# amolchanov86/gym_art

Hardware: AMD Instinct MI355X
Metric: env-steps/sec (whole node) at N=2^20 Hummingbird; achieved HBM GB/s (higher is better)
Workload: dtype f64

## Files before the change

gym_art_amd/_lib.py:

```python
import ctypes as C
import os

import numpy as np

_HERE = os.path.dirname(os.path.abspath(__file__))
LIB_PATH = os.environ.get("GAQ_LIB") or os.path.join(_HERE, "libgaq.so")
ABI_VERSION = 5
STATE_PLANES = 42
AUX_WORDS = 17

CTRL_RAW_ZERO_MIDDLE, CTRL_RAW, CTRL_MELLINGER = 0, 1, 2
NOISE_OFF, NOISE_PHILOX, NOISE_INPUT = 0, 1, 2
REW_QUADROTOR, REW_MULTI_LOG = 0, 1
OBS_BODY_FRAME, OBS_APPEND_H, OBS_APPEND_ACC, OBS_APPEND_ACT = 1, 2, 4, 8
OBS_QUAT, OBS_APPEND_T2W, OBS_APPEND_T2T = 16, 32, 64


class GaqModel(C.Structure):
    _fields_ = [("mass", C.c_double), ("inertia", C.c_double * 3), ("thrust_max", C.c_double * 4),
                ("torque_max", C.c_double * 4), ("prop_pos", C.c_double * 12), ("damp_time_up", C.c_double),
                ("damp_time_down", C.c_double), ("linearity", C.c_double), ("arm", C.c_double),
                ("ou_sigma", C.c_double), ("vel_damp", C.c_double), ("damp_omega_quadratic", C.c_double),
                ("c_drag", C.c_double), ("c_roll", C.c_double)]

# ... 195 lines not shown
    ("gaq_get_aux", C.c_int, [_P, _P]),
    ("gaq_get_state", C.c_int, [_P, _P]),
    ("gaq_set_state", C.c_int, [_P, _P]),
    ("gaq_observe", C.c_int, [_P, _P]),
    ("gaq_done_list", C.c_int, [_P, _P, C.c_int64, C.POINTER(C.c_int64)]),
    ("gaq_set_terminal_obs_dev", C.c_int, [_P, _P]),
    ("gaq_track_episodes", C.c_int, [_P, C.c_int32]),
    ("gaq_episode_stats", C.c_int, [_P, C.POINTER(C.c_int64), C.POINTER(C.c_double), C.POINTER(C.c_double),
                                    C.POINTER(C.c_double), C.c_int32]),
    ("gaq_pack_rows_dev", C.c_int, [_P, _P, _P, _P, _P, _P]),
    ("gaq_set_packed_rows_dev", C.c_int, [_P, _P]),
    ("gaq_nan_count", C.c_int, [_P, C.POINTER(C.c_int64)]),
    ("gaq_last_kernel_ms", C.c_int, [_P, C.POINTER(C.c_float)]),
    ("gaq_set_graph_safe", C.c_int, [_P, C.c_int32]),
    ("gaq_uniform_counters", C.c_int, [_P, C.POINTER(C.c_int32), C.POINTER(C.c_uint32), C.POINTER(C.c_int32)]),
    ("gaq_set_timing", C.c_int, [_P, C.c_int32]),
    ("gaq_hbm_copy_dev", C.c_int, [_P, _P, C.c_size_t, _P]),
    ("gaq_synchronize", C.c_int, [_P]),
    ("gaq_stream", C.c_void_p, [_P]),
    ("gaq_create_sharded", C.c_int, [C.POINTER(GaqConfig), C.POINTER(C.c_int32), C.c_int32, C.POINTER(_P)]),
    ("gaq_sharded_from_handles", C.c_int, [C.POINTER(_P), C.c_int32, C.POINTER(_P)]),
    ("gaq_destroy_sharded", C.c_int, [_P]),
    ("gaq_sharded_num_shards", C.c_int, [_P]),
    ("gaq_sharded_shard", C.c_void_p, [_P, C.c_int32]),
    ("gaq_sharded_range", C.c_int, [_P, C.c_int32, C.POINTER(C.c_int64), C.POINTER(C.c_int64), C.POINTER(C.c_int32)]),
    ("gaq_sharded_num_envs", C.c_int64, [_P]),
    ("gaq_shard_range", C.c_int, [C.c_int64, C.c_int32, C.c_int32, C.c_int32, C.POINTER(C.c_int64), C.POINTER(C.c_int64)]),
    ("gaq_reset_sharded_dev", C.c_int, [_P, _P, _P, _P]),
    ("gaq_step_sharded_dev", C.c_int, [_P, _P, _P, _P, _P, _P]),
    ("gaq_reset_sharded", C.c_int, [_P, _P, _P]),
# ... 100 lines not shown
```

gym_art_amd/csrc/gaq.hip:

```cpp
#include "gaq_host.hpp"

#define GAQ_X(FEAT) extern template __global__ GAQ_STEP_SIG(FEAT)
GAQ_STEP_ALL(GAQ_X)
#undef GAQ_X
#define GAQ_X(FEAT) extern template __global__ GAQ_ROLL_SIG(FEAT)
GAQ_ROLL_ALL(GAQ_X)
#undef GAQ_X

namespace {

using namespace gaqk;

__global__ __launch_bounds__(kBlock) void episode_kernel(int64_t n, const float* __restrict__ reward,
                                                          const uint8_t* __restrict__ done, float* __restrict__ ep_ret,
                                                          uint32_t* __restrict__ ep_len, double* __restrict__ acc) {
  const int64_t i = (int64_t)blockIdx.x * kBlock + threadIdx.x;
  float ret = 0.0f; uint32_t len = 0; bool fin = false;
  if (i < n) {
    ret = ep_ret[i] + reward[i];
    len = ep_len[i] + 1u;
    fin = done[i] != 0;
    ep_ret[i] = fin ? 0.0f : ret;
    ep_len[i] = fin ? 0u : len;
  }
// ... 212 lines not shown
int svd_period_of(double dt) {
  double t = 0.0; int k = 0;
  while (!(t > 0.5)) { t += dt; ++k; if (k > 1000000) break; }
  return k;
}

}

int fail(int code, const std::string& msg) { g_err = msg; return code; }
int env_override(const char* name) { const char* v = getenv(name); return v ? (v[0] == '1' ? 1 : 0) : -1; }
LaunchRecord& launch_record() { static LaunchRecord r; return r; }

namespace {

Overrides read_overrides() {
  return {env_override("GAQ_FORCE_GENERIC") == 1, env_override("GAQ_NO_AUXP") == 1, env_override("GAQ_PREDRAW"), env_override("GAQ_NT"),
          env_override("GAQ_UNIFORM_CTR") != 0};
}
constexpr uint32_t kCtrGuard = 0xA5C3A5C3u;
constexpr int kCtrGuardWords = kTile;
constexpr int kSweepDefault = 1;

struct Layout { bool alias, pack, shadow, fp32; };
struct Selection { uint32_t variant; bool generic; int lds_per_wave; };
struct ParamFlags { bool lag, drag; };
struct Plan { Layout layout; Selection sel; };

bool step_instantiated(uint32_t f) {
  switch (f) {
#define GAQ_X(FEAT) case (FEAT):
    GAQ_STEP_ALL(GAQ_X)
#undef GAQ_X
// ... 363 lines not shown
  }
  const bool self_counting = (launch_variant & gaq::F_CTR) != 0;
  if (e->d.step_ctr && !self_counting) {
    bool capturing = false;
    hipStreamCaptureStatus cs = hipStreamCaptureStatusNone;
    if (hipStreamIsCapturing(st, &cs) == hipSuccess) capturing = cs == hipStreamCaptureStatusActive; else (void)hipGetLastError();
    if (e->ctr_spread || capturing) {
      hipLaunchKernelGGL(fold_counter_kernel, dim3(1), dim3(1), 0, st, e->d.step_ctr);
      HIP_TRY(hipGetLastError());
      if (!capturing) e->ctr_spread = false;
    }
  }
  if (launch_variant != e->noted_step) { launch_record().note(0, launch_variant); e->noted_step = launch_variant; }
#define GAQ_LAUNCH(FEAT) \
  hipLaunchKernelGGL(step_kernel<(FEAT)>, grid, block, lds, st, e->d, e->sc, e->um, actions, obs, reward, done, lpw)
  switch (launch_variant) {
#define GAQ_X(FEAT) case (int)(FEAT): GAQ_LAUNCH(FEAT); break;
    GAQ_STEP_ALL(GAQ_X)
#undef GAQ_X
    default: return fail(GAQ_ERR_STATE, "internal: no kernel instantiation for this feature mask");
  }
#undef GAQ_LAUNCH
  HIP_TRY(hipGetLastError());
  if (e->d.ep_ret) {
    const dim3 g2((unsigned)((e->d.n + kBlock - 1) / kBlock));
    hipLaunchKernelGGL(episode_kernel, g2, block, 0, st, e->d.n, reward, done, e->d.ep_ret, e->d.ep_len, e->d.ep_acc);
    HIP_TRY(hipGetLastError());
  }
  if (e->d.rz_every > 0 && e->d.jinv) { if (int rc = launch_jinv(e, st, done)) return rc; }
  if (e->d.rz_every > 0) {
    e->rz_since_refill += 1;
    const int period = e->sc.ep_len + 1 < 64 ? e->sc.ep_len + 1 : 64;
    if (e->d.step_ctr || e->rz_since_refill >= period) {
// ... 807 lines not shown
  if (!e) return fail(GAQ_ERR_INVALID, "null handle");
  if (valid_out) *valid_out = e->uni.valid ? 1 : 0;
  if (word_out) *word_out = e->uni.word;
  if (guard_intact_out) {
    HIP_TRY(hipSetDevice(e->cfg.device));
    HIP_TRY(hipStreamSynchronize(e->stream));
    if (int rc_ = sync_handle(e)) return rc_;
    uint32_t g[kCtrGuardWords];
    HIP_TRY(hipMemcpy(g, e->d.ctr + e->d.ntiles * kTile, sizeof(g), hipMemcpyDeviceToHost));
    *guard_intact_out = 1;
    for (uint32_t w : g) if (w != kCtrGuard) *guard_intact_out = 0;
  }
  return GAQ_OK;
}

int gaq_set_timing(gaq_env* e, int32_t enabled) {
  if (!e) return fail(GAQ_ERR_INVALID, "null handle");
  e->timing = enabled != 0; e->timed = false;
  return GAQ_OK;
}

int gaq_last_kernel_ms(gaq_env* e, float* ms_out) {
  if (!e || !ms_out) return fail(GAQ_ERR_INVALID, "null argument");
  if (!e->timed) return fail(GAQ_ERR_STATE, "no timed launch recorded (gaq_set_timing)");
  HIP_TRY(hipSetDevice(e->cfg.device));
  HIP_TRY(hipEventSynchronize(e->ev1));
  HIP_TRY(hipEventElapsedTime(ms_out, e->ev0, e->ev1));
  return GAQ_OK;
}

// ... 24 lines not shown
```

gym_art_amd/csrc/gaq_host.hpp:

```cpp
#pragma once

#include <hip/hip_runtime.h>

#include <algorithm>
#include <cmath>
#include <cstdio>
#include <cstdlib>
#include <cstring>
#include <functional>
#include <mutex>
#include <new>
#include <set>
#include <string>
#include <vector>

#include "gaq_kernels.hpp"
#include "../../include/gaq.h"

using namespace gaqk;

namespace {
struct Randomizer {
  int32_t sampler, every;
  double ratio[gaq::TL_COUNT];
  gaq::ParamTree base;
};
}

enum ParamFlag : uint8_t { PF_LAG = 1, PF_DRAG = 2, PF_NONCOMPACT = 4, PF_DAMP = 8 };
inline uint8_t param_flags(double tau_up, double tau_down, double c_drag, double c_roll, bool compact_ok, double vel_damp, double damp_q) {
  return (uint8_t)((!(tau_up >= 1.0 && tau_down >= 1.0) ? PF_LAG : 0) | ((c_drag != 0.0 || c_roll != 0.0) ? PF_DRAG : 0) |
                   (!compact_ok ? PF_NONCOMPACT : 0) | ((vel_damp != 0.0 || damp_q != 0.0) ? PF_DAMP : 0));
}

struct Overrides { bool force_generic = false, no_auxp = false; int predraw = -1, nt = -1; bool uniform_ctr = true; };

struct UniformCtr { bool eligible = false, valid = false, svd_known = false; uint32_t word = 0; };

struct gaq_env {
  gaq_config cfg;
  StepCfg sc;
  Model<double> um;
  DevPtrs d;
  int obs_dim = 18;
  hipStream_t stream = nullptr;
  hipEvent_t ev0 = nullptr, ev1 = nullptr;
  bool timing = false, timed = false;
  uint64_t reset_calls = 0;
  const float* noise_next = nullptr;
  uint32_t noted_step = 0xFFFFFFFFu, noted_roll = 0xFFFFFFFFu, noted_proll = 0xFFFFFFFFu;
// ... 88 lines not shown
```

gym_art_amd/csrc/gaq_inst.hip:

```cpp
#include "gaq_kernels.hpp"

#ifndef GAQ_PART
#error "compile with -DGAQ_PART=0 ... 7"
#endif
#define GAQ_CAT2(a, b) a##b
#define GAQ_CAT(a, b) GAQ_CAT2(a, b)
#define GAQ_X(FEAT) template __global__ GAQ_STEP_SIG(FEAT)
GAQ_CAT(GAQ_STEP_PART, GAQ_PART)(GAQ_X)
#undef GAQ_X
#define GAQ_X(FEAT) template __global__ GAQ_ROLL_SIG(FEAT)
GAQ_CAT(GAQ_ROLL_PART, GAQ_PART)(GAQ_X)
#undef GAQ_X
#define GAQ_X(FEAT) template __global__ GAQ_PROLL_SIG(FEAT)
GAQ_CAT(GAQ_PROLL_PART, GAQ_PART)(GAQ_X)
#undef GAQ_X
```

gym_art_amd/csrc/gaq_kernels.hpp:

```cpp
#pragma once

#include <hip/hip_runtime.h>

#include <cstddef>
#include <cstdint>

#include "../../include/gaq.h"
#include "quad_core.hpp"
#include "quad_params_dev.hpp"

namespace gaqk {

#ifndef GAQ_LD_AUX
#define GAQ_LD_AUX 0
#endif
#ifndef GAQ_ST_AUX
#define GAQ_ST_AUX 0
#endif
#ifndef GAQ_ACT_AUX
#define GAQ_ACT_AUX 0
#endif
#ifndef GAQ_ACTION_AUX
#define GAQ_ACTION_AUX GAQ_ACT_AUX
#endif
// ... 518 lines not shown
  __device__ __forceinline__ void neighbour(int j, const float* me, float* o) const {
    const int src = (int)((lane & ~(uint32_t)(agents - 1)) | ((lane + (uint32_t)j) & (uint32_t)(agents - 1)));
#pragma unroll
    for (int k = 0; k < 6; ++k) o[k] = __shfl(me[k], src);
  }
  __device__ __forceinline__ bool any(bool b) const { return __any(b) != 0; }
};

__device__ __forceinline__ void wait_dma() { asm volatile("s_waitcnt vmcnt(0)" ::: "memory"); }
__device__ __forceinline__ void wave_lds_fence() {
  __builtin_amdgcn_fence(__ATOMIC_RELEASE, "wavefront");
  __builtin_amdgcn_wave_barrier();
  __builtin_amdgcn_fence(__ATOMIC_ACQUIRE, "wavefront");
}

constexpr int kCtrSlots = 64;
constexpr int kCtrStride = 544;
__device__ __forceinline__ uint64_t step_counter_read(const DevPtrs& p, uint32_t lane) {
  static_assert(kCtrSlots == kTile, "one counter word per lane");
  return p.step_ctr[lane * kCtrStride];
}
__device__ __forceinline__ uint64_t step_counter_sum(uint64_t c) {
#pragma unroll
  for (int o = 1; o < kCtrSlots; o <<= 1) c += __shfl_xor(c, o);
  const uint32_t lo = __builtin_amdgcn_readfirstlane((uint32_t)c), hi = __builtin_amdgcn_readfirstlane((uint32_t)(c >> 32));
  return ((uint64_t)hi << 32) | lo;
}
__device__ __forceinline__ uint64_t step_counter_checkin(const DevPtrs& p, uint64_t raw, uint32_t lane) {
  const uint64_t c = step_counter_sum(raw);
  const uint32_t gwave = __builtin_amdgcn_readfirstlane(blockIdx.x * (uint32_t)(kBlock / kTile) + (threadIdx.x >> 6));
// ... 91 lines not shown
    asm("s_waitcnt lgkmcnt(0)" : "+s"(carry) : "s"(token), "s"(p.ntiles), "s"(p.n), "s"(p.step_ctr), "s"(p.ctr_shift), "s"(p.core), "s"(p.ctr),
        "s"(actions), "s"(lds_per_wave));
  }
  return carry;
}

template <uint32_t F> constexpr int kStepMinWaves = 1;
#ifndef GAQ_NO_FLOORS
template <> inline constexpr int kStepMinWaves<214036u> = 3;
template <> inline constexpr int kStepMinWaves<82962u> = 3;
#endif
constexpr uint32_t kXcds = 8;
template <uint32_t F> constexpr bool kSweeps = true;
template <> inline constexpr bool kSweeps<17428u> = false;
template <> inline constexpr bool kSweeps<2569u> = false;
template <uint32_t F>
__global__ __launch_bounds__(kBlock) __attribute__((amdgpu_waves_per_eu(kStepMinWaves<F>))) void step_kernel(DevPtrs p, StepCfg cfg, Model<double> um,
                                                       const float* __restrict__ actions, float* obs,
                                                       float* __restrict__ reward, uint8_t* __restrict__ done,
                                                       int lds_per_wave) {
  constexpr bool G = (F & gaq::F_GENERIC) != 0;
  constexpr bool A = (F & gaq::F_ALIAS) != 0;
  static_assert(!(G && A), "obs/state aliasing exists in the specialised kernels only");
  extern __shared__ __attribute__((aligned(16))) char smem[];
  int wave_ = __builtin_amdgcn_readfirstlane(threadIdx.x >> 6);
  if constexpr (kArgPrologue<F> != 0)
    wave_ = kernarg_batch<F, kArgPrologue<F>, kUniCtr<F>>(kernarg_warm(), wave_, p, actions, lds_per_wave, cfg.sweep);
  const int wave = wave_;
  bool uni = false;
  if constexpr (kUniCtr<F>) uni = ((uint32_t)cfg.sweep & gaq::kUniCtrValid) != 0;
  const uint32_t lane = threadIdx.x & 63u;
  uint32_t block = blockIdx.x;
  if constexpr ((F & gaq::F_CTR) == 0) {
    if (p.step_ctr) cfg.step_index = *p.step_ctr >> p.ctr_shift;
    if constexpr (kSweeps<F>) {
// ... 74 lines not shown
    if constexpr ((F & gaq::F_SWARM) != 0) {
      float* row = reinterpret_cast<float*>(rows) + lane * D;
      gaq::env_step<T, F>(s, *mp, cfg, act, cfg.env_offset + (uint64_t)i, [&](int, int) { return 0.0f; }, out,
                          [&](int k, float v, int) { row[k] = v; }, term_row, WaveSwarm{lane, cfg.swarm.agents});
    } else if constexpr (G) {
      const float* nz = p.noise_in;
      const int64_t n = p.n;
      float* row = reinterpret_cast<float*>(rows) + lane * D;
      if constexpr (kAuxRowsInLds) out.aux_row = reinterpret_cast<float*>(rows + aux_off) + lane * gaq::AUX_WORDS;
      const float* sz = p.sense_in;
      gaq::env_step<T, F>(s, *mp, cfg, act, cfg.env_offset + (uint64_t)i,
                               [&](int k, int c) { return nz[((int64_t)k * 4 + c) * n + i]; }, out,
                               [&](int k, float v, int) { row[k] = v; }, term_row, WaveSwarm{lane, cfg.swarm.agents},
                               [&](int c, int slot, int j) { return sz ? sz[((int64_t)(c * 12 + slot) * 3 + j) * n + i] : 0.0f; });
      if constexpr (gaq::kAux<F> && !kAuxRowsInLds) store_aux(p, i, out);
    } else if constexpr (gaq::kHeadsAreObs<F>) {
      gaq::env_step<T, F>(s, *mp, cfg, act, cfg.env_offset + (uint64_t)i, [&](int k, int c) { return k == 0 ? pre0[c] : pre1[c]; }, out,
                          [&](int, float, int) {}, term_row);
    } else if constexpr (kObsRowsInLds) {
      float* row = reinterpret_cast<float*>(rows) + lane * D;
      if constexpr (kAuxRowsInLds) out.aux_row = reinterpret_cast<float*>(rows + aux_off) + lane * gaq::AUX_WORDS;
      gaq::env_step<T, F>(s, *mp, cfg, act, cfg.env_offset + (uint64_t)i, [&](int, int) { return 0.0f; }, out,
                          [&](int k, float v, int) { row[k] = v; }, term_row);
      if constexpr (gaq::kAux<F> && !kAuxRowsInLds) store_aux(p, i, out);
    } else {
      gaq::env_step<T, F>(s, *mp, cfg, act, cfg.env_offset + (uint64_t)i, [&](int, int) { return 0.0f; }, out,
                          [&](int k, float v, int slot) { if (slot < 0) ob[k] = v; else ob[18 + slot] = v; }, term_row);
      if constexpr (gaq::kAux<F>) store_aux(p, i, out);
    }
  }
// ... 13 lines not shown
        (void)__builtin_amdgcn_raw_ptr_buffer_atomic_add_i32(1, rt, (uint32_t)i * 4u, third, 0);
        (void)__builtin_amdgcn_raw_ptr_buffer_atomic_add_i32(1, rt, (uint32_t)i * 4u, 2 * third, 0);
        s.svd_ctr = 0;
#pragma unroll
        for (int j = 0; j < 4; ++j) s.ou[j] = 0.0f;
      }
    }
  }
  if constexpr (kObsRowsInLds) {
    wave_lds_fence();
    if constexpr (A) flush_obs(p.obs_copy, p.n, D, tile, rows, lane);
    else flush_obs(obs, p.n, D, tile, rows, lane);
    if constexpr (kAuxRowsInLds) { if (p.aux) flush_obs(p.aux, p.n, gaq::AUX_WORDS, tile, rows + aux_off, lane); }
    wave_lds_fence();
  }
  write_image<F>(cfg, buf, lane, s);
  wave_lds_fence();
  stage_out<F>(p, cfg, tile, buf, lane, obs);
  if (!uni) {
    auto rc = __builtin_amdgcn_make_buffer_rsrc(p.ctr, 0, (int)(p.ntiles * kTile * 4), 0x00020000);
    __builtin_amdgcn_raw_buffer_store_b32((s.tick & 0xFFFFu) | (s.svd_ctr << 16), rc, (uint32_t)i * 4u, 0, kStAux<F>);
  }
  if (live) {
    if constexpr (GAQ_OUT_NT != 0) { __builtin_nontemporal_store(out.reward, &reward[i]); __builtin_nontemporal_store(out.done, &done[i]); }
    else { reward[i] = out.reward; done[i] = out.done; }
    if (!isfinite(out.reward)) atomicAdd(p.nan_count, 1u);
  }
  if constexpr (!gaq::kHeadsAreObs<F> && !kObsRowsInLds) {
    float* obs_rows_out = obs;
    if constexpr (A) obs_rows_out = p.obs_copy;
// ... 359 lines not shown
  policy_rollout_body<F>(p, cfg, um, T, obs, reward, done, smem, tile, lane, &pol, scratch, act_out);
}

}

#define GAQ_STEP_PART0(X) X(8u) X(1u) X(3u) X(16u) X(48u) X(2049u) X(2065u) X(3089u) X(2097u) X(4116u) X(8468u) X(16384u) X(33808u) X(197648u) X(459792u) X(197649u) X(199697u) X(16385u) X(16401u) X(18433u) X(18449u)
#define GAQ_STEP_PART1(X) X(9u) X(0u) X(2u) X(17u) X(49u) X(2051u) X(2067u) X(3091u) X(4244u) X(4372u) X(8470u) X(16386u) X(33810u) X(17424u) X(197650u) X(459794u) X(197651u) X(199699u) X(16387u) X(16403u) X(18435u) X(18451u)
#define GAQ_STEP_PART2(X) X(72u) X(2057u) X(4u) X(18u) X(50u) X(2053u) X(2069u) X(3093u) X(4500u) X(4118u) X(8471u) X(16388u) X(33812u) X(66578u) X(66583u) X(68625u) X(16389u) X(16405u) X(18437u) X(18453u)
#define GAQ_STEP_PART3(X) X(73u) X(2121u) X(5u) X(19u) X(51u) X(2055u) X(2071u) X(3095u) X(4246u) X(4374u) X(8596u) X(16390u) X(33814u) X(17426u) X(197652u) X(459796u) X(197653u) X(199701u) X(16391u) X(16407u) X(18439u) X(18455u)
#define GAQ_STEP_PART4(X) X(520u) X(6u) X(20u) X(52u) X(1040u) X(1041u) X(148u) X(276u) X(2099u) X(4502u) X(16400u) X(16402u) X(66576u) X(66581u) X(68627u) X(17425u) X(82960u) X(214032u) X(19473u)
#define GAQ_STEP_PART5(X) X(521u) X(7u) X(21u) X(53u) X(1042u) X(1043u) X(150u) X(278u) X(2101u) X(4119u) X(8598u) X(584u) X(17428u) X(197654u) X(459798u) X(197655u) X(199703u) X(17427u) X(82962u) X(214034u) X(19475u)
#define GAQ_STEP_PART6(X) X(2569u) X(22u) X(54u) X(1044u) X(1045u) X(151u) X(279u) X(404u) X(2103u) X(4247u) X(16404u) X(66580u) X(66577u) X(68631u) X(17429u) X(82964u) X(214036u) X(19477u)
#define GAQ_STEP_PART7(X) X(23u) X(55u) X(1046u) X(1047u) X(406u) X(407u) X(4375u) X(4503u) X(8599u) X(16406u) X(17430u) X(66582u) X(66579u) X(68629u) X(17431u) X(82966u) X(214038u) X(19479u)
#define GAQ_STEP_ALL(X) GAQ_STEP_PART0(X) GAQ_STEP_PART1(X) GAQ_STEP_PART2(X) GAQ_STEP_PART3(X) GAQ_STEP_PART4(X) GAQ_STEP_PART5(X) \
                        GAQ_STEP_PART6(X) GAQ_STEP_PART7(X)
#define GAQ_ROLL_PART0(X) X(16u) X(48u)
#define GAQ_ROLL_PART1(X) X(17u) X(49u)
#define GAQ_ROLL_PART2(X) X(18u) X(50u)
#define GAQ_ROLL_PART3(X) X(19u) X(51u)
#define GAQ_ROLL_PART4(X) X(20u) X(52u)
#define GAQ_ROLL_PART5(X) X(21u) X(53u)
#define GAQ_ROLL_PART6(X) X(22u) X(54u)
#define GAQ_ROLL_PART7(X) X(23u) X(55u)
#define GAQ_ROLL_ALL(X) GAQ_ROLL_PART0(X) GAQ_ROLL_PART1(X) GAQ_ROLL_PART2(X) GAQ_ROLL_PART3(X) GAQ_ROLL_PART4(X) GAQ_ROLL_PART5(X) \
                        GAQ_ROLL_PART6(X) GAQ_ROLL_PART7(X)
#define GAQ_STEP_SIG(FEAT) \
  void gaqk::step_kernel<(FEAT)>(gaqk::DevPtrs, gaq::StepCfg, gaq::Model<double>, const float*, float*, float*, uint8_t*, int);
#define GAQ_PROLL_PART0(X) X(16u) X(48u)
#define GAQ_PROLL_PART1(X) X(17u) X(49u)
#define GAQ_PROLL_PART2(X) X(18u) X(50u)
// ... 12 lines not shown
```

gym_art_amd/csrc/quad_core.hpp:

```cpp
#pragma once

#include <stdint.h>
#include <math.h>

#if defined(__HIPCC__)
#define GAQ_HD __host__ __device__ __forceinline__
#else
#define GAQ_HD inline
#endif

#if defined(__HIP_DEVICE_COMPILE__)
#define GAQ_SINF(x) __sinf(x)
#define GAQ_COSF(x) __cosf(x)
#define GAQ_LOGF(x) __logf(x)
#ifndef GAQ_REWARD_SQRT_FAST
#define GAQ_REWARD_SQRT_FAST 1
#endif
#if GAQ_REWARD_SQRT_FAST
#define GAQ_SQRTF_OUT(x) __builtin_amdgcn_sqrtf(x)
#else
#define GAQ_SQRTF_OUT(x) sqrtf(x)
#endif
#else
#define GAQ_SINF(x) sinf(x)
// ... 146 lines not shown
}
template <uint32_t F> GAQ_HD int swarm_agents(const StepCfg& c) { if constexpr (kSwarm<F>) return c.swarm.agents; else return 0; }
template <uint32_t F> constexpr bool kGyroBias = ((F & F_GENERIC) != 0 && (F & F_LITE) == 0) || (F & F_BIAS) != 0;
template <uint32_t F> GAQ_HD bool has_gyro_bias(const StepCfg& c) { if constexpr (kGyroBias<F>) return c.gyro_bias != 0; else return false; }

template <typename T>
struct EnvState {
  T pos[3], vel[3], rot[9], omega[3];
  T rot_damp[4];
  float cmds_damp[4];
  float ou[4];
  float act_prev[4];
  T goal[3];
  float gyro_bias[3];
  uint32_t tick, svd_ctr;
};

struct StepOut {
  float reward;
  uint8_t done, crashed;
  float acc_meter[3];
  float omega_dot[3], torque[3], ctrl[4], cmds[4];
  float* aux_row = nullptr;
};
enum { AUX_ACC = 0, AUX_OMEGA_DOT = 3, AUX_TORQUE = 6, AUX_CTRL = 9, AUX_CMDS = 13, AUX_WORDS = 17 };

GAQ_HD double clampv(double x, double lo, double hi) { return fmin(fmax(x, lo), hi); }
GAQ_HD float clampv(float x, float lo, float hi) { return fminf(fmaxf(x, lo), hi); }
GAQ_HD double sqrt_t(double x) { return sqrt(x); }
GAQ_HD float sqrt_t(float x) { return sqrtf(x); }
// ... 220 lines not shown
      cr[j] = s.omega[j] + dt * wd;                                                                                  \
    }                                                                                                                \
  }                                                                                                                  \
  _Pragma("unroll") for (int j = 0; j < 3; ++j) s.omega[j] = clampv(cr[j], T(-40), T(40));
template <typename T, bool EXACT>
GAQ_HD void euler_omega(EnvState<T>& s, const Model<T>& m, T dt, const T tq[3], bool first_after_reset, T wd_out[3]) {
  if constexpr (EXACT) {
#pragma clang fp contract(off)
    GAQ_OMEGA_BODY(cross3_nofma)
  } else {
    GAQ_OMEGA_BODY(cross3)
  }
}
#undef GAQ_OMEGA_BODY

template <typename T, uint32_t F>
GAQ_HD void step1(EnvState<T>& s, const Model<T>& m, const StepCfg& cfg, const T u[4], const T w[4],
                  const float nrm[4], bool first_after_reset, float* acc_meter, StepOut* aux = nullptr) {
  constexpr bool G = (F & F_GENERIC) != 0;
  const T dt = T(cfg.dt);
  T c[4];
  model_fence<F>();
  if (has_lag<F>(cfg)) {
#pragma clang fp contract(off)
#pragma unroll
    for (int i = 0; i < 4; ++i) {
      const T prev = (noise_mode<F>(cfg) == NOISE_OFF) ? s.rot_damp[i] * s.rot_damp[i] : T(s.cmds_damp[i]);
      T tau = (u[i] < prev) ? m.tau_down : m.tau_up;
      tau = tau > T(1) ? T(1) : tau;
      s.rot_damp[i] = tau * (w[i] - s.rot_damp[i]) + s.rot_damp[i];
      c[i] = s.rot_damp[i] * s.rot_damp[i];
    }
  } else {
#pragma unroll
    for (int i = 0; i < 4; ++i) c[i] = u[i];
  }
  if (noise_mode<F>(cfg) != NOISE_OFF) {
#pragma unroll
    for (int i = 0; i < 4; ++i) {
      s.ou[i] = s.ou[i] + (0.15f * (0.0f - s.ou[i]) + m.ou_sigma * nrm[i]);
      c[i] = clampv(c[i] + u[i] * T(s.ou[i]), T(0), T(1));
    }
  } else {
#pragma unroll
    for (int i = 0; i < 4; ++i) c[i] = clampv(c[i], T(0), T(1));
  }
  if (has_lag<F>(cfg)) {
#pragma unroll
    for (int i = 0; i < 4; ++i) s.cmds_damp[i] = (float)c[i];
  }
  constexpr bool EXACT = (F & (F_LAG | F_PER_ENV | F_GENERIC | F_MELL)) != 0;
  T tq[3] = {T(0), T(0), T(0)};
  T fz = T(0);
  model_fence<F>();
  thrust_torque<T, EXACT>(m, c, tq, fz);
  model_fence<F>();
// ... 73 lines not shown
    if (aux) {
      if constexpr (kAuxIsRow<F>) {
#pragma unroll
        for (int j = 0; j < 3; ++j) { aux->aux_row[AUX_OMEGA_DOT + j] = (float)wd[j]; aux->aux_row[AUX_TORQUE + j] = (float)tq[j]; }
#pragma unroll
        for (int j = 0; j < 4; ++j) aux->aux_row[AUX_CMDS + j] = (float)c[j];
      } else {
#pragma unroll
        for (int j = 0; j < 3; ++j) { aux->omega_dot[j] = (float)wd[j]; aux->torque[j] = (float)tq[j]; }
#pragma unroll
        for (int j = 0; j < 4; ++j) aux->cmds[j] = (float)c[j];
      }
    }
  }
  {
    const T* R = s.rot;
    T acc[3];
#pragma unroll
    for (int j = 0; j < 3; ++j) {
      s.pos[j] = clampv(s.pos[j] + dt * s.vel[j], T(cfg.room_lo[j]), T(cfg.room_hi[j]));
      T f = R[3 * j + 2] * (fz + drag_f[2]);
      if constexpr (G && (F & F_LITE) == 0) f = R[3 * j] * drag_f[0] + R[3 * j + 1] * drag_f[1] + f;
      acc[j] = m.inv_mass * f;
    }
    acc[2] += T(-9.81);
    if (m.vel_damp != T(0)) {
#pragma unroll
      for (int j = 0; j < 3; ++j) s.vel[j] = (T(1) - m.vel_damp) * s.vel[j] + dt * acc[j];
    } else {
#pragma unroll
// ... 346 lines not shown
      const double fn = 1.0 / sqrt(fw[0] * fw[0] + fw[1] * fw[1] + fw[2] * fw[2]);
      fw[0] *= fn; fw[1] *= fn; fw[2] *= fn;
      double lf[3] = {up[1] * fw[2] - up[2] * fw[1], up[2] * fw[0] - up[0] * fw[2], up[0] * fw[1] - up[1] * fw[0]};
      const double ln = 1.0 / sqrt(lf[0] * lf[0] + lf[1] * lf[1] + lf[2] * lf[2]);
      lf[0] *= ln; lf[1] *= ln; lf[2] *= ln;
      const double u2[3] = {fw[1] * lf[2] - fw[2] * lf[1], fw[2] * lf[0] - fw[0] * lf[2], fw[0] * lf[1] - fw[1] * lf[0]};
#pragma unroll
      for (int j = 0; j < 3; ++j) { s.rot[3 * j] = T(fw[j]); s.rot[3 * j + 1] = T(lf[j]); s.rot[3 * j + 2] = T(u2[j]); }
    }
  }
#pragma unroll
  for (int i = 0; i < 4; ++i) { s.rot_damp[i] = T(0); s.cmds_damp[i] = 0.0f; s.act_prev[i] = 0.0f; }
  s.tick = 0;
}

template <typename T, uint32_t F, typename NormalSrc, typename Sink, typename Swarm = NoSwarm, typename SenseSrc = NoSense>
GAQ_HD void env_step(EnvState<T>& s, const Model<T>& m, const StepCfg& cfg, const float action[4], uint64_t env_global,
                     NormalSrc&& get_normal, StepOut& out, Sink&& put_obs, float* term_row = nullptr, Swarm&& sw = NoSwarm(),
                     SenseSrc&& get_sense = NoSense()) {
  constexpr bool G = (F & F_GENERIC) != 0;
  float hist1[4] = {0.0f, 0.0f, 0.0f, 0.0f};
  if (has_act_prev<F>(cfg)) {
#pragma unroll
    for (int i = 0; i < 4; ++i) hist1[i] = s.act_prev[i];
  }
  if constexpr (kEnvExtras<F>) {
    if (cfg.excite && (s.tick % 5u) == 0u) {
      const Philox e(cfg.seed, env_global, cfg.step_index, RNG_EXCITE);
      s.goal[0] = T((float)(e.u01(0) - 0.5)); s.goal[1] = T((float)(e.u01(1) - 0.5)); s.goal[2] = T((float)(1.5 + e.u01(2)));
    }
  }
  T t2w = T(0), t2t = T(0);
  if constexpr (kAux<F>) {
    if (cfg.obs_flags & (OBS_APPEND_T2W | OBS_APPEND_T2T)) {
// ... 20 lines not shown
        if constexpr (kAuxIsRow<F>) out.aux_row[AUX_CTRL + i] = (float)cmd[i]; else out.ctrl[i] = (float)cmd[i];
      }
    }
  }
  T u[4], w[4];
#pragma unroll
  for (int i = 0; i < 4; ++i) {
    u[i] = clampv(cmd[i], T(0), T(1));
    w[i] = has_lag<F>(cfg) ? sqrt_t(u[i]) : T(0);
  }
  const bool fresh = (s.tick == 0);
  const float poison = (float)(((s.pos[0] + s.pos[1] + s.pos[2]) + (s.vel[0] + s.vel[1] + s.vel[2]) +
                                (s.omega[0] + s.omega[1] + s.omega[2])) * T(0)) +
                       ((action[0] + action[1]) + (action[2] + action[3])) * 0.0f;
  out.acc_meter[0] = 0.0f; out.acc_meter[1] = 0.0f; out.acc_meter[2] = (float)cfg.gravity;
  for (int k = 0; k < cfg.sim_steps; ++k) {
    float nrm[4] = {0.0f, 0.0f, 0.0f, 0.0f};
    const int nm = noise_mode<F>(cfg);
    if (nm == NOISE_PHILOX) {
      bool have = false;
      if constexpr ((F & F_PREDRAW) != 0) {
        if (k < 2) {
#pragma unroll
          for (int i = 0; i < 4; ++i) nrm[i] = get_normal(k, i);
          have = true;
        }
      }
      if (!have) {
        const Philox r(cfg.seed, env_global, cfg.step_index, RNG_OU0 + (uint32_t)k);
        normals4(r, nrm);
      }
    } else if (nm == NOISE_INPUT) {
#pragma unroll
      for (int i = 0; i < 4; ++i) nrm[i] = get_normal(k, i);
    }
    float* am = nullptr;
    if constexpr (!kHeadsAreObs<F>) am = (((cfg.obs_flags & OBS_APPEND_ACC) || want_aux) && k == cfg.sim_steps - 1) ? out.acc_meter : nullptr;
    StepOut* auxp = nullptr;
    if constexpr (kAux<F>) auxp = (want_aux && k == cfg.sim_steps - 1) ? &out : nullptr;
    step1<T, F>(s, m, cfg, u, w, nrm, fresh && k == 0, am, auxp);
  }
  float swarm_penalty = 0.0f;
  if constexpr (kSwarm<F>) {
    if (cfg.swarm.agents > 1) {
      float dv[3];
      swarm_penalty = swarm_interact(s, cfg, sw, dv);
      if (cfg.swarm.response) {
#pragma unroll
        for (int j = 0; j < 3; ++j) s.vel[j] += T(dv[j]);
      }
    }
  }
  const bool crashed = s.pos[2] <= m.arm;
  out.crashed = crashed;
  out.reward = reward<T, F>(s, cfg, action, hist1, crashed) + poison;
  if constexpr (kSwarm<F>) out.reward -= (float)cfg.dt * swarm_penalty;
  if (s.tick < 0xFFFFu) s.tick += 1;
  const bool done = s.tick > (uint32_t)cfg.ep_len;
  out.done = done;
  if (has_act_prev<F>(cfg)) {
#pragma unroll
    for (int i = 0; i < 4; ++i) s.act_prev[i] = action[i];
  }
  if constexpr (kSwarm<F>) {
    if (cfg.swarm.agents > 1 && sw.any(cfg.auto_reset && done && term_row != nullptr)) {
      const bool wr = cfg.auto_reset && done && term_row != nullptr;
      pack_obs<T, F>(s, cfg, out.acc_meter, hist1, [&](int k, float v, int) { if (wr) term_row[k] = v; }, env_global,
                     cfg.step_index ^ (1ull << 62), 3, sw, get_sense, t2w, t2t);
    }
// ... 29 lines not shown
```

include/gaq.h:

```cpp
#ifndef GAQ_H
#define GAQ_H

#include <stddef.h>
#include <stdint.h>

#ifdef __cplusplus
extern "C" {
#endif

#define GAQ_ABI_VERSION 5

typedef struct gaq_env gaq_env;

typedef enum gaq_status {
  GAQ_OK = 0,
  GAQ_ERR_INVALID = -1,
  GAQ_ERR_DEVICE = -2,
  GAQ_ERR_NAN = -3,
  GAQ_ERR_STATE = -4
} gaq_status;

enum { GAQ_CTRL_RAW_ZERO_MIDDLE = 0, GAQ_CTRL_RAW = 1, GAQ_CTRL_MELLINGER = 2 };
enum { GAQ_NOISE_OFF = 0, GAQ_NOISE_PHILOX = 1, GAQ_NOISE_INPUT = 2 };
enum { GAQ_REW_QUADROTOR = 0, GAQ_REW_MULTI_LOG = 1 };
// ... 424 lines not shown
                      int32_t clear);

int gaq_done_list(gaq_env* env, uint32_t* idx_out, int64_t capacity, int64_t* count_out);

int gaq_pack_rows_dev(gaq_env* env, const float* obs_dev, const float* reward_dev, const uint8_t* done_dev, float* rows_dev,
                      void* stream);

int gaq_set_packed_rows_dev(gaq_env* env, float* rows_dev_or_null);

int gaq_nan_count(gaq_env* env, int64_t* count_out);

int gaq_set_graph_safe(gaq_env* env, int32_t enabled);

int gaq_uniform_counters(gaq_env* env, int32_t* valid_out, uint32_t* word_out, int32_t* guard_intact_out);

int gaq_last_kernel_ms(gaq_env* env, float* ms_out);
int gaq_set_timing(gaq_env* env, int32_t enabled);

int gaq_hbm_copy_dev(void* dst_dev, const void* src_dev, size_t bytes, void* stream);

int gaq_synchronize(gaq_env* env);
void* gaq_stream(gaq_env* env);

typedef struct gaq_sharded gaq_sharded;
int gaq_create_sharded(const gaq_config* cfg, const int32_t* device_ids, int32_t num_devices, gaq_sharded** out);
int gaq_sharded_from_handles(gaq_env* const* envs, int32_t num_shards, gaq_sharded** out);
int gaq_destroy_sharded(gaq_sharded* s);
int gaq_sharded_num_shards(const gaq_sharded* s);
gaq_env* gaq_sharded_shard(gaq_sharded* s, int32_t k);
int gaq_sharded_range(const gaq_sharded* s, int32_t k, int64_t* first, int64_t* count, int32_t* device);
// ... 13 lines not shown
```

Baseline: 22.73 billion.

## Park step state in idle LDS tile image to run four waves per EU

```diff
diff --git a/gym_art_amd/_lib.py b/gym_art_amd/_lib.py
--- a/gym_art_amd/_lib.py
+++ b/gym_art_amd/_lib.py
@@ -233,6 +233,7 @@
     ("gaq_last_kernel_ms", C.c_int, [_P, C.POINTER(C.c_float)]),
     ("gaq_set_graph_safe", C.c_int, [_P, C.c_int32]),
     ("gaq_uniform_counters", C.c_int, [_P, C.POINTER(C.c_int32), C.POINTER(C.c_uint32), C.POINTER(C.c_int32)]),
+    ("gaq_step_form", C.c_int, [_P, C.POINTER(C.c_int32), C.POINTER(C.c_int32)]),
     ("gaq_set_timing", C.c_int, [_P, C.c_int32]),
     ("gaq_hbm_copy_dev", C.c_int, [_P, _P, C.c_size_t, _P]),
     ("gaq_synchronize", C.c_int, [_P]),
diff --git a/gym_art_amd/csrc/gaq.hip b/gym_art_amd/csrc/gaq.hip
--- a/gym_art_amd/csrc/gaq.hip
+++ b/gym_art_amd/csrc/gaq.hip
@@ -2,6 +2,7 @@
 
 #define GAQ_X(FEAT) extern template __global__ GAQ_STEP_SIG(FEAT)
 GAQ_STEP_ALL(GAQ_X)
+GAQ_STEP_W4(GAQ_X)
 #undef GAQ_X
 #define GAQ_X(FEAT) extern template __global__ GAQ_ROLL_SIG(FEAT)
 GAQ_ROLL_ALL(GAQ_X)
@@ -250,8 +251,19 @@
 namespace {
 
 Overrides read_overrides() {
+  const char* waves = getenv("GAQ_STEP_WAVES");
   return {env_override("GAQ_FORCE_GENERIC") == 1, env_override("GAQ_NO_AUXP") == 1, env_override("GAQ_PREDRAW"), env_override("GAQ_NT"),
-          env_override("GAQ_UNIFORM_CTR") != 0};
+          env_override("GAQ_UNIFORM_CTR") != 0, waves && waves[0] == '3' && waves[1] == 0};
+}
+uint32_t step_form_of(uint32_t launch_variant, const Overrides& ov) {
+  if (ov.three_waves) return launch_variant;
+  switch (launch_variant | kFormW4) {
+#define GAQ_X(FEAT) case (FEAT):
+    GAQ_STEP_W4(GAQ_X)
+#undef GAQ_X
+      return launch_variant | kFormW4;
+    default: return launch_variant;
+  }
 }
 constexpr uint32_t kCtrGuard = 0xA5C3A5C3u;
 constexpr int kCtrGuardWords = kTile;
@@ -645,9 +657,10 @@
   if (launch_variant != e->noted_step) { launch_record().note(0, launch_variant); e->noted_step = launch_variant; }
 #define GAQ_LAUNCH(FEAT) \
   hipLaunchKernelGGL(step_kernel<(FEAT)>, grid, block, lds, st, e->d, e->sc, e->um, actions, obs, reward, done, lpw)
-  switch (launch_variant) {
+  switch (step_form_of(launch_variant, e->ov)) {
 #define GAQ_X(FEAT) case (int)(FEAT): GAQ_LAUNCH(FEAT); break;
     GAQ_STEP_ALL(GAQ_X)
+    GAQ_STEP_W4(GAQ_X)
 #undef GAQ_X
     default: return fail(GAQ_ERR_STATE, "internal: no kernel instantiation for this feature mask");
   }
@@ -1485,6 +1498,14 @@
   return GAQ_OK;
 }
 
+int gaq_step_form(const gaq_env* e, int32_t* waves_out, int32_t* override_out) {
+  if (!e) return fail(GAQ_ERR_INVALID, "null handle");
+  const uint32_t v = launch_variant_of(e);
+  if (waves_out) *waves_out = step_form_of(v, Overrides()) == v ? 0 : step_form_of(v, e->ov) == v ? 3 : 4;
+  if (override_out) *override_out = e->ov.three_waves ? 3 : 0;
+  return GAQ_OK;
+}
+
 int gaq_set_timing(gaq_env* e, int32_t enabled) {
   if (!e) return fail(GAQ_ERR_INVALID, "null handle");
   e->timing = enabled != 0; e->timed = false;
diff --git a/gym_art_amd/csrc/gaq_host.hpp b/gym_art_amd/csrc/gaq_host.hpp
--- a/gym_art_amd/csrc/gaq_host.hpp
+++ b/gym_art_amd/csrc/gaq_host.hpp
@@ -33,7 +33,8 @@
                    (!compact_ok ? PF_NONCOMPACT : 0) | ((vel_damp != 0.0 || damp_q != 0.0) ? PF_DAMP : 0));
 }
 
-struct Overrides { bool force_generic = false, no_auxp = false; int predraw = -1, nt = -1; bool uniform_ctr = true; };
+struct Overrides { bool force_generic = false, no_auxp = false; int predraw = -1, nt = -1; bool uniform_ctr = true;
+                   bool three_waves = false; };
 
 struct UniformCtr { bool eligible = false, valid = false, svd_known = false; uint32_t word = 0; };
 
diff --git a/gym_art_amd/csrc/gaq_inst.hip b/gym_art_amd/csrc/gaq_inst.hip
--- a/gym_art_amd/csrc/gaq_inst.hip
+++ b/gym_art_amd/csrc/gaq_inst.hip
@@ -7,6 +7,9 @@
 #define GAQ_CAT(a, b) GAQ_CAT2(a, b)
 #define GAQ_X(FEAT) template __global__ GAQ_STEP_SIG(FEAT)
 GAQ_CAT(GAQ_STEP_PART, GAQ_PART)(GAQ_X)
+#if GAQ_PART == 4
+GAQ_STEP_W4(GAQ_X)
+#endif
 #undef GAQ_X
 #define GAQ_X(FEAT) template __global__ GAQ_ROLL_SIG(FEAT)
 GAQ_CAT(GAQ_ROLL_PART, GAQ_PART)(GAQ_X)
diff --git a/gym_art_amd/csrc/gaq_kernels.hpp b/gym_art_amd/csrc/gaq_kernels.hpp
--- a/gym_art_amd/csrc/gaq_kernels.hpp
+++ b/gym_art_amd/csrc/gaq_kernels.hpp
@@ -556,6 +556,15 @@
   __builtin_amdgcn_fence(__ATOMIC_ACQUIRE, "wavefront");
 }
 
+struct LdsPark {
+  static constexpr bool on = true;
+  uint32_t* mine;
+  template <typename S> __device__ __forceinline__ static LdsPark of(const S& s) { return LdsPark{s.park}; }
+  __device__ __forceinline__ void put(int slot, uint32_t v) const { mine[slot * kTile] = v; }
+  __device__ __forceinline__ uint32_t get(int slot) const { return mine[slot * kTile]; }
+  __device__ __forceinline__ void fence() const { wave_lds_fence(); }
+};
+
 constexpr int kCtrSlots = 64;
 constexpr int kCtrStride = 544;
 __device__ __forceinline__ uint64_t step_counter_read(const DevPtrs& p, uint32_t lane) {
@@ -677,11 +686,17 @@
 template <uint32_t F> constexpr bool kSweeps = true;
 template <> inline constexpr bool kSweeps<17428u> = false;
 template <> inline constexpr bool kSweeps<2569u> = false;
+constexpr uint32_t kFormW4 = 524288u;
+template <> inline constexpr int kStepMinWaves<148u | kFormW4> = 4;
+template <> inline constexpr int kStepMinWaves<20u | kFormW4> = 4;
 template <uint32_t F>
 __global__ __launch_bounds__(kBlock) __attribute__((amdgpu_waves_per_eu(kStepMinWaves<F>))) void step_kernel(DevPtrs p, StepCfg cfg, Model<double> um,
                                                        const float* __restrict__ actions, float* obs,
                                                        float* __restrict__ reward, uint8_t* __restrict__ done,
                                                        int lds_per_wave) {
+  constexpr bool PARK = (F & kFormW4) != 0;
+  static_assert(!PARK || (kStepMinWaves<F> == 4 && gaq::kHeadsAreObs<F> && kRowsLds + kLoRowsLds >= gaq::PARK_SLOTS * kTile * 4),
+                "parking: the tile image is idle, and large enough, in the heads-are-the-observation kernels");
   constexpr bool G = (F & gaq::F_GENERIC) != 0;
   constexpr bool A = (F & gaq::F_ALIAS) != 0;
   static_assert(!(G && A), "obs/state aliasing exists in the specialised kernels only");
@@ -786,6 +801,13 @@
                                [&](int k, float v, int) { row[k] = v; }, term_row, WaveSwarm{lane, cfg.swarm.agents},
                                [&](int c, int slot, int j) { return sz ? sz[((int64_t)(c * 12 + slot) * 3 + j) * n + i] : 0.0f; });
       if constexpr (gaq::kAux<F> && !kAuxRowsInLds) store_aux(p, i, out);
+    } else if constexpr (PARK) {
+      s.park = reinterpret_cast<uint32_t*>(buf) + lane;
+      if constexpr ((F & gaq::F_PREDRAW) != 0) gaq::park_put_n<4>(LdsPark::of(s), gaq::PARK_NRM1, pre1);
+      auto first_normals = [&](int, int c) { return pre0[c]; };
+      auto no_sink = [&](int, float, int) {};
+      gaq::env_step<T, F, decltype(first_normals)&, decltype(no_sink)&, gaq::NoSwarm, gaq::NoSense, LdsPark>(
+          s, *mp, cfg, act, cfg.env_offset + (uint64_t)i, first_normals, out, no_sink, term_row);
     } else if constexpr (gaq::kHeadsAreObs<F>) {
       gaq::env_step<T, F>(s, *mp, cfg, act, cfg.env_offset + (uint64_t)i, [&](int k, int c) { return k == 0 ? pre0[c] : pre1[c]; }, out,
                           [&](int, float, int) {}, term_row);
@@ -829,6 +851,7 @@
     if constexpr (kAuxRowsInLds) { if (p.aux) flush_obs(p.aux, p.n, gaq::AUX_WORDS, tile, rows + aux_off, lane); }
     wave_lds_fence();
   }
+  if constexpr (PARK) wave_lds_fence();
   write_image<F>(cfg, buf, lane, s);
   wave_lds_fence();
   stage_out<F>(p, cfg, tile, buf, lane, obs);
@@ -1218,6 +1241,8 @@
 #define GAQ_STEP_PART7(X) X(23u) X(55u) X(1046u) X(1047u) X(406u) X(407u) X(4375u) X(4503u) X(8599u) X(16406u) X(17430u) X(66582u) X(66579u) X(68629u) X(17431u) X(82966u) X(214038u) X(19479u)
 #define GAQ_STEP_ALL(X) GAQ_STEP_PART0(X) GAQ_STEP_PART1(X) GAQ_STEP_PART2(X) GAQ_STEP_PART3(X) GAQ_STEP_PART4(X) GAQ_STEP_PART5(X) \
                         GAQ_STEP_PART6(X) GAQ_STEP_PART7(X)
+#define GAQ_STEP_W4(X) X(524436u) X(524308u)
+static_assert((148u | gaqk::kFormW4) == 524436u && (20u | gaqk::kFormW4) == 524308u, "GAQ_STEP_W4");
 #define GAQ_ROLL_PART0(X) X(16u) X(48u)
 #define GAQ_ROLL_PART1(X) X(17u) X(49u)
 #define GAQ_ROLL_PART2(X) X(18u) X(50u)
diff --git a/gym_art_amd/csrc/quad_core.hpp b/gym_art_amd/csrc/quad_core.hpp
--- a/gym_art_amd/csrc/quad_core.hpp
+++ b/gym_art_amd/csrc/quad_core.hpp
@@ -184,6 +184,7 @@
   T goal[3];
   float gyro_bias[3];
   uint32_t tick, svd_ctr;
+  uint32_t* park;
 };
 
 struct StepOut {
@@ -434,9 +435,37 @@
 }
 #undef GAQ_OMEGA_BODY
 
-template <typename T, uint32_t F>
+enum { PARK_POS = 0, PARK_VEL = 6, PARK_ACT = 12, PARK_NRM1 = 16, PARK_OU = 20, PARK_SLOTS = 24 };
+struct NoPark {
+  static constexpr bool on = false;
+  template <typename S> GAQ_HD static NoPark of(const S&) { return NoPark(); }
+  GAQ_HD void put(int, uint32_t) const {}
+  GAQ_HD uint32_t get(int) const { return 0u; }
+  GAQ_HD void fence() const {}
+};
+template <typename P> GAQ_HD void park_put(const P& pk, int slot, float v) { pk.put(slot, __builtin_bit_cast(uint32_t, v)); }
+template <typename P> GAQ_HD void park_put(const P& pk, int slot, double v) {
+  const uint64_t b = __builtin_bit_cast(uint64_t, v);
+  pk.put(slot, (uint32_t)b); pk.put(slot + 1, (uint32_t)(b >> 32));
+}
+template <typename P> GAQ_HD void park_get(const P& pk, int slot, float& v) { v = __builtin_bit_cast(float, pk.get(slot)); }
+template <typename P> GAQ_HD void park_get(const P& pk, int slot, double& v) {
+  const uint32_t lo = pk.get(slot), hi = pk.get(slot + 1);
+  v = __builtin_bit_cast(double, ((uint64_t)hi << 32) | lo);
+}
+template <int N, typename P, typename V> GAQ_HD void park_put_n(const P& pk, int slot, const V* v) {
+#pragma unroll
+  for (int j = 0; j < N; ++j) park_put(pk, slot + j * (int)(sizeof(V) / 4), v[j]);
+}
+template <int N, typename P, typename V> GAQ_HD void park_get_n(const P& pk, int slot, V* v) {
+#pragma unroll
+  for (int j = 0; j < N; ++j) park_get(pk, slot + j * (int)(sizeof(V) / 4), v[j]);
+}
+
+template <typename T, uint32_t F, typename Park = NoPark>
 GAQ_HD void step1(EnvState<T>& s, const Model<T>& m, const StepCfg& cfg, const T u[4], const T w[4],
                   const float nrm[4], bool first_after_reset, float* acc_meter, StepOut* aux = nullptr) {
+  const Park pk = Park::of(s);
   constexpr bool G = (F & F_GENERIC) != 0;
   const T dt = T(cfg.dt);
   T c[4];
@@ -455,11 +484,28 @@
 #pragma unroll
     for (int i = 0; i < 4; ++i) c[i] = u[i];
   }
+  if constexpr (Park::on) {
+    park_put_n<3>(pk, PARK_POS, s.pos); park_put_n<3>(pk, PARK_VEL, s.vel);
+    pk.fence();
+  }
   if (noise_mode<F>(cfg) != NOISE_OFF) {
+    if constexpr (Park::on) {
+      park_get_n<4>(pk, PARK_OU, s.ou);
+#pragma unroll
+      for (int i = 0; i < 4; ++i) {
+#pragma clang fp contract(off)
+        const float drawn = m.ou_sigma * nrm[i];
+        s.ou[i] = s.ou[i] + __builtin_fmaf(0.0f - s.ou[i], 0.15f, drawn);
+      }
+      park_put_n<4>(pk, PARK_OU, s.ou);
+#pragma unroll
+      for (int i = 0; i < 4; ++i) c[i] = clampv(c[i] + u[i] * T(s.ou[i]), T(0), T(1));
+    } else {
 #pragma unroll
     for (int i = 0; i < 4; ++i) {
       s.ou[i] = s.ou[i] + (0.15f * (0.0f - s.ou[i]) + m.ou_sigma * nrm[i]);
       c[i] = clampv(c[i] + u[i] * T(s.ou[i]), T(0), T(1));
+    }
     }
   } else {
 #pragma unroll
@@ -563,6 +609,10 @@
     }
   }
   {
+    if constexpr (Park::on) {
+      pk.fence();
+      park_get_n<3>(pk, PARK_POS, s.pos); park_get_n<3>(pk, PARK_VEL, s.vel);
+    }
     const T* R = s.rot;
     T acc[3];
 #pragma unroll
@@ -939,10 +989,13 @@
   s.tick = 0;
 }
 
-template <typename T, uint32_t F, typename NormalSrc, typename Sink, typename Swarm = NoSwarm, typename SenseSrc = NoSense>
+template <typename T, uint32_t F, typename NormalSrc, typename Sink, typename Swarm = NoSwarm, typename SenseSrc = NoSense,
+          typename Park = NoPark>
 GAQ_HD void env_step(EnvState<T>& s, const Model<T>& m, const StepCfg& cfg, const float action[4], uint64_t env_global,
                      NormalSrc&& get_normal, StepOut& out, Sink&& put_obs, float* term_row = nullptr, Swarm&& sw = NoSwarm(),
                      SenseSrc&& get_sense = NoSense()) {
+  const Park pk = Park::of(s);
+  static_assert(!Park::on || (kHeadsAreObs<F> && (F & (F_PER_ENV | F_LAG | F_FP32)) == 0), "parking: the heads-are-the-observation kernels");
   constexpr bool G = (F & F_GENERIC) != 0;
   float hist1[4] = {0.0f, 0.0f, 0.0f, 0.0f};
   if (has_act_prev<F>(cfg)) {
@@ -993,6 +1046,13 @@
                                 (s.omega[0] + s.omega[1] + s.omega[2])) * T(0)) +
                        ((action[0] + action[1]) + (action[2] + action[3])) * 0.0f;
   out.acc_meter[0] = 0.0f; out.acc_meter[1] = 0.0f; out.acc_meter[2] = (float)cfg.gravity;
+  if constexpr (Park::on) {
+#if defined(__HIP_DEVICE_COMPILE__)
+    asm volatile("" :: "v"(poison));
+#endif
+    park_put_n<4>(pk, PARK_ACT, action);
+    if (noise_mode<F>(cfg) != NOISE_OFF) park_put_n<4>(pk, PARK_OU, s.ou);
+  }
   for (int k = 0; k < cfg.sim_steps; ++k) {
     float nrm[4] = {0.0f, 0.0f, 0.0f, 0.0f};
     const int nm = noise_mode<F>(cfg);
@@ -1000,8 +1060,17 @@
       bool have = false;
       if constexpr ((F & F_PREDRAW) != 0) {
         if (k < 2) {
-#pragma unroll
-          for (int i = 0; i < 4; ++i) nrm[i] = get_normal(k, i);
+          if constexpr (Park::on) {
+            if (k == 1) {
+              park_get_n<4>(pk, PARK_NRM1, nrm);
+            } else {
+#pragma unroll
+              for (int i = 0; i < 4; ++i) nrm[i] = get_normal(0, i);
+            }
+          } else {
+#pragma unroll
+            for (int i = 0; i < 4; ++i) nrm[i] = get_normal(k, i);
+          }
           have = true;
         }
       }
@@ -1017,7 +1086,11 @@
     if constexpr (!kHeadsAreObs<F>) am = (((cfg.obs_flags & OBS_APPEND_ACC) || want_aux) && k == cfg.sim_steps - 1) ? out.acc_meter : nullptr;
     StepOut* auxp = nullptr;
     if constexpr (kAux<F>) auxp = (want_aux && k == cfg.sim_steps - 1) ? &out : nullptr;
-    step1<T, F>(s, m, cfg, u, w, nrm, fresh && k == 0, am, auxp);
+    step1<T, F, Park>(s, m, cfg, u, w, nrm, fresh && k == 0, am, auxp);
+  }
+  if constexpr (Park::on) {
+    pk.fence();
+    if (noise_mode<F>(cfg) != NOISE_OFF) park_get_n<4>(pk, PARK_OU, s.ou);
   }
   float swarm_penalty = 0.0f;
   if constexpr (kSwarm<F>) {
@@ -1032,6 +1105,11 @@
   }
   const bool crashed = s.pos[2] <= m.arm;
   out.crashed = crashed;
+  if constexpr (Park::on) {
+    float back[4];
+    park_get_n<4>(pk, PARK_ACT, back);
+    out.reward = reward<T, F>(s, cfg, back, hist1, crashed) + poison;
+  } else
   out.reward = reward<T, F>(s, cfg, action, hist1, crashed) + poison;
   if constexpr (kSwarm<F>) out.reward -= (float)cfg.dt * swarm_penalty;
   if (s.tick < 0xFFFFu) s.tick += 1;
diff --git a/include/gaq.h b/include/gaq.h
--- a/include/gaq.h
+++ b/include/gaq.h
@@ -462,6 +462,8 @@
 
 int gaq_uniform_counters(gaq_env* env, int32_t* valid_out, uint32_t* word_out, int32_t* guard_intact_out);
 
+int gaq_step_form(const gaq_env* env, int32_t* waves_out, int32_t* override_out);
+
 int gaq_last_kernel_ms(gaq_env* env, float* ms_out);
 int gaq_set_timing(gaq_env* env, int32_t enabled);
 
```

Result: no change. 22.66 billion (-0.3%).
